# RTCartist/Neuromorphic-Spatiotemporal-Optical-Flow

Hardware: AMD Instinct MI355X
Metric: 1080p frame-pairs/sec (Farneback, HIP) (higher is better)
Workload: dtype f32

## Files before the change

neuromorphic-spatiotemporal-optical-flow_amd/csrc/farneback_iterate_x.hip:

```cpp
#include "iterate_common.h"

namespace {

typedef __attribute__((address_space(1))) unsigned long long gu64;
typedef __attribute__((address_space(1))) unsigned gu32;
typedef __attribute__((address_space(3))) int lds_int;

__device__ __forceinline__ unsigned xcc_id() { return __builtin_amdgcn_s_getreg(20 | (0 << 6) | (3 << 11)) & 7u; }

template <int MH>
struct XGeom {
    static constexpr int COLS = 208, NCW = 3, RB = 4;
    static constexpr int RL = 2 * MH + 1 + 2 * RB;
    static constexpr int HALO = 2 * MH + 1;
    static constexpr int SW = NCW * 64;
    static_assert(SW + HALO <= COLS && SW % 8 == 0, "strip geometry");
    static constexpr int NB = COLS / 64, REM = COLS % 64;
    static_assert(REM == 16, "the remainder wave maps 4 rows x 16 columns onto its 64 lanes");
    static constexpr int SEG0 = 96, SEG1 = SW - SEG0;
    static_assert(SEG0 % 8 == 0 && SEG1 % 8 == 0 && SEG0 >= SEG1 && SEG1 > 0, "segments: whole 8-column blocks, the left one not shorter");
    static constexpr int SVW = SW + 2;
    static constexpr int WAVES = NCW + 1 + 2 * NB + 1 + 1;
    static constexpr int THREADS = 64 * WAVES;
    static constexpr int CQ = 1, IOQ = 1;
    static constexpr size_t SV1_BYTES = sizeof(double) * 4 * 5 * SVW;
    static constexpr size_t SV_BYTES = 2 * SV1_BYTES;
    static constexpr size_t VI_BYTES = sizeof(double) * 2 * 4 * 5 * MH;
    static constexpr size_t JOB_BYTES = 16;
    static constexpr size_t CB_BYTES = sizeof(double) * 2 * 2 * 20;
    static constexpr size_t RING4_BYTES = sizeof(float) * 4 * RL * COLS, RING1_BYTES = sizeof(float) * RL * COLS;
    static constexpr size_t SMEM = SV_BYTES + VI_BYTES + JOB_BYTES + CB_BYTES + RING4_BYTES + RING1_BYTES;
};

struct XRing {
    float4* q;
    float* c;
    int cols;
    __device__ __forceinline__ void put(int slot, int col, const float (&M)[5]) const
    {
        q[slot * cols + col] = make_float4(M[0], M[1], M[2], M[3]);
        c[slot * cols + col] = M[4];
    }
    __device__ __forceinline__ void get(int slot, int col, float (&M)[5]) const
    {
        const float4 v = q[slot * cols + col];
        M[0] = v.x; M[1] = v.y; M[2] = v.z; M[3] = v.w;
        M[4] = c[slot * cols + col];
    }
};

constexpr unsigned X_SPIN_LIMIT = 1u << 21;

template <int MH>
__device__ __forceinline__ void x_produce(RowIn& in, float2& fl, const XRing& ring, const Planes& R0,
                                          const Planes& R1, const FlowSrc& F, int W, int H, int xc, int col, int i)
{
    constexpr int RL = XGeom<MH>::RL;
    float Mn[5];
    matrix_from(in, xc, min(i, H - 1), W, H, Mn);
    ring.put((i + MH + 1) % RL, col, Mn);
    issue_row(in, R0, R1, W, H, xc, min(i + 8, H - 1), fl);
    fl = F.fetch(min(i + 16, H - 1));
}

template <int MH>
__device__ __forceinline__ void x_rows_above(const XRing& ring, const Planes& R0, const Planes& R1, const FlowSrc& F,
                                             int W, int H, int xc, int col)
{
    float2 fl[MH];
#pragma unroll
    for (int i = 0; i < MH; i++) fl[i] = F.fetch(min(i, H - 1));
    constexpr int GRP = 4;
#pragma unroll
    for (int g0 = 0; g0 < MH; g0 += GRP) {
        RowIn t[GRP];
#pragma unroll
        for (int k = 0; k < GRP; k++)
            if (g0 + k < MH) issue_row(t[k], R0, R1, W, H, xc, min(g0 + k, H - 1), fl[g0 + k]);
#pragma unroll
        for (int k = 0; k < GRP; k++)
            if (g0 + k < MH) {
                float Mi[5];
                matrix_from(t[k], xc, min(g0 + k, H - 1), W, H, Mi);
                if (g0 + k == 0) {
#pragma unroll
                    for (int j = 0; j <= MH + 1; j++) ring.put(j, col, Mi);
                } else {
                    ring.put(g0 + k + MH + 1, col, Mi);
                }
            }
    }
}

template <int MH, int GP>
__device__ __forceinline__ void x_producer_loop(const XRing& ring, const Planes& R0, const Planes& R1,
                                                const FlowSrc& F, int W, int H, int xc, int col, int nimg)
{
    if constexpr (GP == 0) x_rows_above<MH>(ring, R0, R1, F, W, H, xc, col);
    RowIn in[2][2];
    float2 fl[2][2];
#pragma unroll
    for (int ts = 0; ts < 2; ts++)
#pragma unroll
        for (int rr = 0; rr < 2; rr++) {
            const int r = min(4 * ts + MH + 2 * GP + rr, H - 1);
            issue_row(in[ts][rr], R0, R1, W, H, xc, r, F.fetch(r));
        }
#pragma unroll
    for (int ts = 0; ts < 2; ts++)
#pragma unroll
        for (int rr = 0; rr < 2; rr++) fl[ts][rr] = F.fetch(min(4 * (ts + 2) + MH + 2 * GP + rr, H - 1));
    auto step = [&](auto tsc, int t) {
        constexpr int TS = decltype(tsc)::value;
        x_produce<MH>(in[TS][0], fl[TS][0], ring, R0, R1, F, W, H, xc, col, 4 * t + MH + 2 * GP);
        x_produce<MH>(in[TS][1], fl[TS][1], ring, R0, R1, F, W, H, xc, col, 4 * t + MH + 2 * GP + 1);
    };
    step(std::integral_constant<int, 0>{}, 0);
    __syncthreads();
    step(std::integral_constant<int, 1>{}, 1);
    __syncthreads();
    for (int t = 0; t <= nimg; t += 2) {
        step(std::integral_constant<int, 0>{}, t + 2);
        __syncthreads();
        if (t + 1 > nimg) break;
        step(std::integral_constant<int, 1>{}, t + 3);
        __syncthreads();
    }
}

template <int MH, int Q0, int NQ>
__device__ __forceinline__ void x_solve_rows(const double* sv, volatile lds_int* flag, float2* Fout, size_t fpitch, int W, int H,
                                             int x0, int nimg, double scale, int lane, int t)
{
    using G = XGeom<MH>;
    constexpr int SVW = G::SVW, NBLK = G::SW / 64;
    double g[NBLK][NQ][5];
    int us[NBLK];
#pragma unroll
    for (int b = 0; b < NBLK; b++) {
        const int col = b * 64 + lane;
        const int u = t - 1 - (col >= G::SEG0 ? 1 : 0);
        us[b] = (u >= 0 && u < nimg && x0 + col < W) ? u : -1;
        const double* p = sv + (u & 1) * (G::SV1_BYTES / sizeof(double)) + col;
#pragma unroll
        for (int q = 0; q < NQ; q++)
#pragma unroll
            for (int c = 0; c < 5; c++) g[b][q][c] = p[((q + Q0) * 5 + c) * SVW];
    }
    asm volatile("s_waitcnt lgkmcnt(0)" ::: "memory");
    if (lane == 0) *flag = t + 1;
#pragma unroll
    for (int b = 0; b < NBLK; b++) {
        if (us[b] < 0) continue;
        const int x = x0 + b * 64 + lane;
#pragma unroll
        for (int q = 0; q < NQ; q++) {
            const int yo = 4 * us[b] + q + Q0;
            const double g11 = g[b][q][0] * scale, g12 = g[b][q][1] * scale, g22 = g[b][q][2] * scale;
            const double h1 = g[b][q][3] * scale, h2 = g[b][q][4] * scale;
            const double idet = nsof_recip_normal(g11 * g22 - g12 * g12 + 1e-3);
            const float ox = (float)((g11 * h2 - g12 * h1) * idet), oy = (float)((g22 * h1 - g12 * h2) * idet);
            if (yo < H) nsof_store_stream2(reinterpret_cast<float*>(Fout + (size_t)yo * fpitch + x), ox, oy);
        }
    }
}

template <int MH>
__device__ __forceinline__ void x_remainder_loop(const XRing& ring, double* cb, const Planes& R0, const Planes& R1,
                                                 const FlowSrc& F, int W, int H, int xc, int col, int r, int nimg,
                                                 gu64* cin, gu64* cout, unsigned epoch, gu32* err, const double* sv,
                                                 volatile lds_int* ioflag, float2* Fout, size_t fpitch, int x0, double scale)
{
    const int lane = threadIdx.x & 63;
    const bool io = lane < 20;
    const int l = io ? lane : 0;
    unsigned long long g0 = 0, g1 = 0;
    auto carry_load = [&](int s) {
        const gu64* q = cin + 40 * s + 2 * l;
        asm volatile("global_load_dwordx2 %0, %2, off sc1\n\tglobal_load_dwordx2 %1, %2, off offset:8 sc1"
                     : "=&v"(g0), "=&v"(g1) : "v"(q) : "memory");
    };
    auto fetch_issue = [&](int s) {
        if (!cin || !io) return;
        carry_load(s);
    };
    bool dead = false;
    auto fetch_finish = [&](int s) {
        if (!cin || !io) return;
        asm volatile("s_waitcnt vmcnt(9)" : "+v"(g0), "+v"(g1) : : "memory");
        for (unsigned spins = 0; !dead; spins++) {
            if (__all((unsigned)(g0 >> 32) == epoch && (unsigned)(g1 >> 32) == epoch)) break;
            if (spins > X_SPIN_LIMIT ||
                ((spins & 255u) == 255u && __hip_atomic_load(err, __ATOMIC_RELAXED, __HIP_MEMORY_SCOPE_AGENT) != 0u)) {
                if (lane == 0) __hip_atomic_fetch_or(err, 1u, __ATOMIC_RELAXED, __HIP_MEMORY_SCOPE_AGENT);
                dead = true;
                break;
            }
            __builtin_amdgcn_s_sleep(8);
            carry_load(s);
            asm volatile("s_waitcnt vmcnt(0)" : "+v"(g0), "+v"(g1) : : "memory");
        }
        cb[40 + (s & 1) * 20 + l] = __hiloint2double((int)(unsigned)g1, (int)(unsigned)g0);
    };
    auto publish = [&](int s) {
        if (!cout || !io) return;
        const double S = cb[(s & 1) * 20 + l];
        const unsigned long long tag = (unsigned long long)epoch << 32;
        __hip_atomic_store(cout + 40 * s + 2 * l, tag | (unsigned)__double2loint(S), __ATOMIC_RELAXED, __HIP_MEMORY_SCOPE_AGENT);
        __hip_atomic_store(cout + 40 * s + 2 * l + 1, tag | (unsigned)__double2hiint(S), __ATOMIC_RELAXED, __HIP_MEMORY_SCOPE_AGENT);
    };
    if (r == 0) x_rows_above<MH>(ring, R0, R1, F, W, H, xc, col);
    RowIn in[2];
    float2 fl[2];
#pragma unroll
    for (int ts = 0; ts < 2; ts++) {
        const int y = min(4 * ts + MH + r, H - 1);
        issue_row(in[ts], R0, R1, W, H, xc, y, F.fetch(y));
    }
#pragma unroll
    for (int ts = 0; ts < 2; ts++) fl[ts] = F.fetch(min(4 * (ts + 2) + MH + r, H - 1));
    x_produce<MH>(in[0], fl[0], ring, R0, R1, F, W, H, xc, col, MH + r);
    __syncthreads();
    fetch_issue(0);
    x_produce<MH>(in[1], fl[1], ring, R0, R1, F, W, H, xc, col, 4 + MH + r);
    fetch_finish(0);
    __syncthreads();
    auto window = [&](auto tsc, int t) {
        constexpr int TS = decltype(tsc)::value;
        if (t >= 2) publish(t - 2);
        if (t + 1 < nimg) fetch_issue(t + 1);
        x_produce<MH>(in[TS], fl[TS], ring, R0, R1, F, W, H, xc, col, 4 * (t + 2) + MH + r);
        x_solve_rows<MH, XGeom<MH>::CQ, XGeom<MH>::IOQ>(sv, ioflag, Fout, fpitch, W, H, x0, nimg, scale, lane, t);
        if (t + 1 < nimg) fetch_finish(t + 1);
        __syncthreads();
    };
    for (int t = 0; t <= nimg; t += 2) {
        window(std::integral_constant<int, 0>{}, t);
        if (t + 1 > nimg) break;
        window(std::integral_constant<int, 1>{}, t + 1);
    }
    publish(nimg - 1);
    x_solve_rows<MH, XGeom<MH>::CQ, XGeom<MH>::IOQ>(sv, ioflag, Fout, fpitch, W, H, x0, nimg, scale, lane, nimg + 1);
}

template <int MH>
__device__ __forceinline__ void x_consumer_loop(const XRing& ring, double* sv, double* vinit, volatile lds_int* sflag, float2* Fout,
                                                size_t fpitch, int W, int H, int x0, int j, int nimg, double scale, bool strip0)
{
    using G = XGeom<MH>;
    constexpr int RL = G::RL, SVW = G::SVW, HALO = G::HALO;
    const int rb = j, ra = j + HALO;
    const int vik = j == 0 ? 0 : j - MH - 1;
    const bool vi_thread = strip0 && (j == 0 || (j >= MH + 2 && j <= 2 * MH));
    __syncthreads();
    double va[5], vb[5];
    {
        float a0[5], b0[5];
        ring.get(MH + 1, ra, a0);
        ring.get(MH + 1, rb, b0);
#pragma unroll
        for (int c = 0; c < 5; c++) {
            va[c] = (double)(a0[c] * (float)(MH + 2));
            vb[c] = (double)(b0[c] * (float)(MH + 2));
        }
#pragma unroll
        for (int i = 1; i < MH; i++) {
            ring.get(i + MH + 1, ra, a0);
            ring.get(i + MH + 1, rb, b0);
#pragma unroll
            for (int c = 0; c < 5; c++) {
                va[c] += (double)a0[c];
                vb[c] += (double)b0[c];
            }
        }
    }
    int slot_new = (2 * MH + 1) % RL;
    int slot_old = 0;
    const int x = x0 + j;
    const int lag = j >= G::SEG0 ? 1 : 0;
    double D[2][4][5];
    auto column_sums = [&](auto pc, int s) {
        constexpr int P = decltype(pc)::value;
#pragma unroll
        for (int q = 0; q < 4; q++) {
            float na[5], oa[5], nb[5], ob[5];
            ring.get(slot_new, ra, na);
            ring.get(slot_old, ra, oa);
            ring.get(slot_new, rb, nb);
            ring.get(slot_old, rb, ob);
#pragma unroll
            for (int c = 0; c < 5; c++) {
                const float da = na[c] - oa[c];
                const float db = nb[c] - ob[c];
                va[c] += (double)da;
                vb[c] += (double)db;
                D[P][q][c] = va[c] - vb[c];
            }
            if (vi_thread) {
#pragma unroll
                for (int c = 0; c < 5; c++) vinit[(((s & 1) * 4 + q) * 5 + c) * MH + vik] = vb[c];
            }
            slot_new = slot_new + 1 == RL ? 0 : slot_new + 1;
            slot_old = slot_old + 1 == RL ? 0 : slot_old + 1;
        }
    };
    auto publish = [&](auto pc, int p) {
        constexpr int P = decltype(pc)::value;
        if (p < 0 || p >= nimg) return;
        double* svj = sv + (p & 1) * (G::SV1_BYTES / sizeof(double)) + j;
#pragma unroll
        for (int q = 0; q < 4; q++)
#pragma unroll
            for (int c = 0; c < 5; c++) svj[(q * 5 + c) * SVW] = D[P][q][c];
    };
    column_sums(std::integral_constant<int, 0>{}, 0);
    if (!lag) publish(std::integral_constant<int, 0>{}, 0);
    __syncthreads();
    auto window = [&](auto pc, int t) {
        constexpr int P = decltype(pc)::value;
        const int u = t - 1 - lag;
        if (u >= 0 && u < nimg && x < W) {
            const double* svj = sv + (u & 1) * (G::SV1_BYTES / sizeof(double)) + j;
#pragma unroll
            for (int q = 0; q < G::CQ; q++) {
                const int yo = 4 * u + q;
                const double g11 = svj[(q * 5 + 0) * SVW] * scale, g12 = svj[(q * 5 + 1) * SVW] * scale;
                const double g22 = svj[(q * 5 + 2) * SVW] * scale;
                const double h1 = svj[(q * 5 + 3) * SVW] * scale, h2 = svj[(q * 5 + 4) * SVW] * scale;
                const double idet = nsof_recip_normal(g11 * g22 - g12 * g12 + 1e-3);
                const float ox = (float)((g11 * h2 - g12 * h1) * idet), oy = (float)((g22 * h1 - g12 * h2) * idet);
                if (yo < H) nsof_store_stream2(reinterpret_cast<float*>(Fout + (size_t)yo * fpitch + x), ox, oy);
            }
        }
        if (t == nimg + 1) return;
        if (t + 1 < nimg) column_sums(std::integral_constant<int, P ^ 1>{}, t + 1);
        for (int spin = 0; (sflag[0] < t + 1 || sflag[1] < t + 1) && spin < (1 << 22); spin++)
            __builtin_amdgcn_s_sleep(1);
        if (lag) publish(std::integral_constant<int, P>{}, t);
        else publish(std::integral_constant<int, P ^ 1>{}, t + 1);
        __syncthreads();
    };
    for (int t = 0; t <= nimg + 1; t += 2) {
        window(std::integral_constant<int, 0>{}, t);
        if (t + 1 > nimg + 1) break;
        window(std::integral_constant<int, 1>{}, t + 1);
    }
}

template <int MH>
__device__ __forceinline__ void x_solver_loop(const double* sv, volatile lds_int* sflag, float2* Fout, size_t fpitch, int W, int H,
                                              int x0, int nimg, double scale, int lane)
{
    using G = XGeom<MH>;
    __syncthreads();
    __syncthreads();
    for (int t = 0; t <= nimg + 1; t++) {
        x_solve_rows<MH, G::CQ + G::IOQ, 4 - G::CQ - G::IOQ>(sv, sflag, Fout, fpitch, W, H, x0, nimg, scale, lane, t);
        if (t <= nimg) __syncthreads();
    }
}

template <int MH>
__device__ __forceinline__ void x_scanner_loop(double* sv, const double* vinit, double* cb, bool has_left, int nimg, int ncols,
                                               int lane)
{
    using G = XGeom<MH>;
    constexpr int SVW = G::SVW;
    typedef double d2 __attribute__((ext_vector_type(2)));
    const int seg = lane >= 20 ? 1 : 0;
    const int l = lane < 40 ? lane - 20 * seg : 0;
    double Smid = 0.;
    __syncthreads();
    __builtin_amdgcn_s_setprio(3);
    __syncthreads();
    for (int t = 0; t <= nimg; t++) {
        const int step = t - seg;
        const double Sleft = __shfl(Smid, lane >= 20 ? lane - 20 : lane);
        d2* row = reinterpret_cast<d2*>(sv + (step & 1) * (G::SV1_BYTES / sizeof(double)) + l * SVW + seg * G::SEG0);
        if (lane < 40 && step >= 0 && step < nimg) {
            double S;
            if (seg) {
                S = Sleft;
            } else if (has_left) {
                S = cb[40 + (step & 1) * 20 + l];
            } else {
                const double* vi = vinit + ((step & 1) * 20 + l) * MH;
                S = vi[0] * (double)(MH + 2);
#pragma unroll
                for (int k = 1; k < MH; k++) S += vi[k];
            }
            auto scan_blocks = [&](int b0, int nb) {
                unsigned a = (unsigned)(size_t)(__attribute__((address_space(3))) char*)(row + 4 * b0);
                int nrem = nb - 1;
                asm volatile(
                "ds_read_b128 v[64:67], %[a]\n\t"
                "ds_read_b128 v[68:71], %[a] offset:16\n\t"
                "ds_read_b128 v[72:75], %[a] offset:32\n\t"
                "ds_read_b128 v[76:79], %[a] offset:48\n\t"
                "ds_read_b128 v[80:83], %[a] offset:64\n\t"
                "ds_read_b128 v[84:87], %[a] offset:80\n\t"
                "ds_read_b128 v[88:91], %[a] offset:96\n\t"
                "ds_read_b128 v[92:95], %[a] offset:112\n\t"
                "s_waitcnt lgkmcnt(7)\n\t"
                "v_add_f64 v[64:65], %[S], v[64:65]\n\t"
                "v_add_f64 v[66:67], v[66:67], v[64:65]\n\t"
                "s_waitcnt lgkmcnt(6)\n\t"
                "v_add_f64 v[68:69], v[66:67], v[68:69]\n\t"
                "v_add_f64 v[70:71], v[70:71], v[68:69]\n\t"
                "s_waitcnt lgkmcnt(5)\n\t"
                "v_add_f64 v[72:73], v[70:71], v[72:73]\n\t"
// ... 51 lines not shown
                "ds_write_b128 %[a], v[68:71] offset:144\n\t"
                "ds_write_b128 %[a], v[72:75] offset:160\n\t"
                "ds_write_b128 %[a], v[76:79] offset:176\n\t"
                "v_add_u32 %[a], 128, %[a]\n\t"
                "s_sub_i32 %[n], %[n], 2\n\t"
                "s_cmp_ge_i32 %[n], 2\n\t"
                "s_cbranch_scc1 .Lxs_loop%=\n"
                ".Lxs_tail%=:\n\t"
                "s_cmp_lt_i32 %[n], 1\n\t"
                "s_cbranch_scc1 .Lxs_done%=\n\t"
                "s_waitcnt lgkmcnt(4)\n\t"
                "v_add_f64 v[80:81], v[78:79], v[80:81]\n\t"
                "v_add_f64 v[82:83], v[82:83], v[80:81]\n\t"
                "s_waitcnt lgkmcnt(4)\n\t"
                "v_add_f64 v[84:85], v[82:83], v[84:85]\n\t"
                "v_add_f64 v[86:87], v[86:87], v[84:85]\n\t"
                "s_waitcnt lgkmcnt(4)\n\t"
                "v_add_f64 v[88:89], v[86:87], v[88:89]\n\t"
                "v_add_f64 v[90:91], v[90:91], v[88:89]\n\t"
                "s_waitcnt lgkmcnt(4)\n\t"
                "v_add_f64 v[92:93], v[90:91], v[92:93]\n\t"
                "v_add_f64 v[94:95], v[94:95], v[92:93]\n\t"
                "s_nop 1\n\t"
                "ds_write_b128 %[a], v[80:83] offset:64\n\t"
                "ds_write_b128 %[a], v[84:87] offset:80\n\t"
                "ds_write_b128 %[a], v[88:91] offset:96\n\t"
                "ds_write_b128 %[a], v[92:95] offset:112\n\t"
                "v_mov_b64 v[78:79], v[94:95]\n"
                ".Lxs_done%=:\n\t"
                "v_mov_b64 %[S], v[78:79]\n\t"
                "s_waitcnt lgkmcnt(0)\n\t"
                    : [S] "+v"(S), [a] "+v"(a), [n] "+s"(nrem)
                    :
                    : "memory", "scc", "v64", "v65", "v66", "v67", "v68", "v69", "v70", "v71", "v72", "v73", "v74", "v75", "v76", "v77", "v78", "v79", "v80", "v81", "v82", "v83", "v84", "v85", "v86", "v87", "v88", "v89", "v90", "v91", "v92", "v93", "v94", "v95");
            };
            const int nb0 = ncols >> 3, nba = nb0 < G::SEG1 / 8 ? nb0 : G::SEG1 / 8;
            scan_blocks(0, nba);
            if (nb0 > nba && !seg) scan_blocks(nba, nb0 - nba);
            if (seg) cb[(step & 1) * 20 + l] = S;
            else Smid = S;
        }
        __syncthreads();
    }
}

template <int MH, bool HET>
__global__ __launch_bounds__((XGeom<MH>::THREADS)) void k_iterate_x(
    const float* __restrict__ R0b, const float* __restrict__ R1b, size_t pair_stride, const float* __restrict__ flow_in,
    float* __restrict__ flow_out, int W, int H, int block_size, const nsof_het_item* __restrict__ items, int het_final,
    int n, int nstrips, unsigned long long* carry, unsigned* tickets, unsigned epoch, unsigned* err, int fault,
    const unsigned* __restrict__ xjobs)
{
    using G = XGeom<MH>;
    constexpr int SW = G::SW, COLS = G::COLS;
    extern __shared__ __attribute__((aligned(16))) unsigned char smem_x[];
    double* sv = reinterpret_cast<double*>(smem_x);
    double* vinit = reinterpret_cast<double*>(smem_x + G::SV_BYTES);
    int* job = reinterpret_cast<int*>(smem_x + G::SV_BYTES + G::VI_BYTES);
    double* cb = reinterpret_cast<double*>(smem_x + G::SV_BYTES + G::VI_BYTES + G::JOB_BYTES);
    XRing ring;
    ring.q = reinterpret_cast<float4*>(smem_x + G::SV_BYTES + G::VI_BYTES + G::JOB_BYTES + G::CB_BYTES);
    ring.c = reinterpret_cast<float*>(smem_x + G::SV_BYTES + G::VI_BYTES + G::JOB_BYTES + G::CB_BYTES + G::RING4_BYTES);
    ring.cols = COLS;
    const int tid = threadIdx.x;
    if (tid == 0) {
        const unsigned share = HET ? 0u : (unsigned)((n + 7) / 8) * (unsigned)nstrips;
        unsigned k = xcc_id();
        unsigned lim = HET ? xjobs[k] : share;
        unsigned i = __hip_atomic_fetch_add(tickets + 32 * k, 1u, __ATOMIC_RELAXED, __HIP_MEMORY_SCOPE_AGENT);
        if (__hip_atomic_load((gu32*)err, __ATOMIC_RELAXED, __HIP_MEMORY_SCOPE_AGENT) != 0u) i = 0xffffffffu, lim = 0;
        else if (i >= lim) {
            for (unsigned d = 1; d < 8 && i >= lim; d++) {
                k = (k + 1) & 7u;
                if constexpr (HET) lim = xjobs[k];
                i = __hip_atomic_fetch_add(tickets + 32 * k, 1u, __ATOMIC_RELAXED, __HIP_MEMORY_SCOPE_AGENT);
            }
        }
        if constexpr (HET) {
            const unsigned e = i < lim ? xjobs[8u + k * (unsigned)nstrips + i] : 0xffffffffu;
            job[0] = e != 0xffffffffu ? (int)(e >> 8) : -1;
            job[1] = (int)(e & 255u);
        } else {
            job[0] = i < share ? (int)((i / (unsigned)nstrips) * 8u + k) : -1;
            job[1] = (int)(i % (unsigned)nstrips);
        }
        job[2] = job[3] = 0;
    }
    __syncthreads();
    const int pair = job[0], strip = job[1];
    if (pair < 0 || pair >= n) return;
    size_t fpitch = (size_t)W;
    gu64* cbase;
    if constexpr (HET) {
        const nsof_het_item& it = items[pair];
        W = it.wk;
        H = it.hk;
        if (strip * SW >= W) return;
        R0b += it.offR;
        R1b = R0b + 5 * (size_t)W * H;
        pair_stride = 0;
        flow_in += 2 * it.offF;
        cbase = (gu64*)(carry + it.offR / 2);
        if (het_final) {
            flow_out = it.out;
            fpitch = (size_t)it.out_pitch;
        } else {
            flow_out += 2 * it.offF;
            fpitch = (size_t)W;
        }
    } else {
        if (strip * SW >= W) return;
        cbase = (gu64*)(carry + (size_t)pair * nstrips * (size_t)(((H + 3) / 4) * 40));
    }
    const int nimg = (H + 3) / 4;
    const int x0 = strip * SW;
    const size_t plane = (size_t)W * H;
    const size_t poff = HET ? 0 : (size_t)pair * pair_stride;
    const Planes R0 = planes_of(R0b + poff, plane);
    const Planes R1 = planes_of(R1b + poff, plane);
    const int wave = __builtin_amdgcn_readfirstlane(tid >> 6);
    volatile lds_int* sflag = (volatile lds_int*)(job + 2);
    if (wave < G::NCW) {
        float2* Fout = reinterpret_cast<float2*>(flow_out) + (HET ? 0 : (size_t)pair * plane);
        x_consumer_loop<MH>(ring, sv, vinit, sflag, Fout, fpitch, W, H, x0, tid, nimg, 1. / (block_size * block_size), strip == 0);
    } else if (wave == G::WAVES - 1) {
        float2* Fout = reinterpret_cast<float2*>(flow_out) + (HET ? 0 : (size_t)pair * plane);
        x_solver_loop<MH>(sv, sflag, Fout, fpitch, W, H, x0, nimg, 1. / (block_size * block_size), tid & 63);
    } else if (wave == G::NCW) {
        const int ncols = min(G::SEG0, (W - x0 + 7) & ~7);
        x_scanner_loop<MH>(sv, vinit, cb, strip > 0, nimg, ncols, tid & 63);
    } else {
        const int pw = wave - (G::NCW + 1);
        const int lane = tid & 63;
        FlowSrc F;
        F.base = reinterpret_cast<const char*>(flow_in) + (HET ? 0 : (size_t)pair * plane * 8);
        F.W = (unsigned)W;
        const bool is_io = pw == G::NB;
        const int gp = pw < G::NB ? 0 : 1;
        const int blk = pw < G::NB ? pw : pw - G::NB - 1;
        if (is_io) {
            const int col = G::NB * 64 + (lane & 15), r = lane >> 4;
            const int xc = clampi(x0 - MH - 1 + col, 0, W - 1);
            F.xc = (unsigned)xc;
            const size_t per_strip = (size_t)nimg * 40;
            gu64* cin = strip > 0 ? cbase + (size_t)(strip - 1) * per_strip : nullptr;
            gu64* cout = x0 + SW < W && !((fault & 1) && pair == 0 && strip == 0) ? cbase + (size_t)strip * per_strip : nullptr;
            float2* Fout = reinterpret_cast<float2*>(flow_out) + (HET ? 0 : (size_t)pair * plane);
            x_remainder_loop<MH>(ring, cb, R0, R1, F, W, H, xc, col, r, nimg, cin, cout, epoch, (gu32*)err, sv, sflag + 1, Fout, fpitch,
                                 x0, 1. / (block_size * block_size));
        } else {
            const int col = blk * 64 + lane;
            const int xc = clampi(x0 - MH - 1 + col, 0, W - 1);
            F.xc = (unsigned)xc;
            if (gp == 0)
                x_producer_loop<MH, 0>(ring, R0, R1, F, W, H, xc, col, nimg);
            else
                x_producer_loop<MH, 1>(ring, R0, R1, F, W, H, xc, col, nimg);
        }
    }
}

template <int MH, bool HET>
int launch_x(nsof_ctx* ctx, int n, int max_w, int max_h, const float* R0, const float* R1, size_t pair_stride,
             const float* flow_in, float* flow_out, int W, int H, int winsize, const nsof_het_item* items, bool final,
             const unsigned* xjobs, int stride, int njobs)
{
    using G = XGeom<MH>;
    static_assert(G::SW == NSOF_X_STRIP, "the host's job tables count strips of NSOF_X_STRIP columns");
    if (int rc = lds_opt_in(ctx, k_iterate_x<MH, HET>, G::SMEM)) return rc;
    const int nstrips = HET ? stride : (max_w + G::SW - 1) / G::SW;
    unsigned long long* carry = nullptr;
    unsigned* tickets = nullptr;
    unsigned* err = nullptr;
    const size_t cbytes = HET ? 0 : (size_t)n * nstrips * (size_t)((max_h + 3) / 4) * 40 * 8;
    if (int rc = nsof_xsync_reserve(ctx, cbytes, &carry, &tickets, &err)) return rc;
    NSOF_HIP(ctx, hipMemsetAsync(tickets, 0, 8 * 32 * sizeof(unsigned), ctx->stream));
    unsigned epoch = ++ctx->x_epoch;
    if (epoch == 0) {
        NSOF_HIP(ctx, hipMemsetAsync(ctx->x_carry, 0, ctx->x_carry_bytes, ctx->stream));
        epoch = ++ctx->x_epoch;
    }
    const unsigned grid = HET ? (unsigned)njobs : 8u * (unsigned)((n + 7) / 8) * (unsigned)nstrips;
    hipLaunchKernelGGL((k_iterate_x<MH, HET>), dim3(grid), dim3(G::THREADS), G::SMEM, ctx->stream, R0, R1, pair_stride, flow_in,
                       flow_out, W, H, winsize, items, final ? 1 : 0, n, nstrips, carry, tickets, epoch, err, ctx->dbg_fault,
                       xjobs);
    return NSOF_OK;
}

}

bool nsof_iterate_x_supported(int winsize, int W, int H)
{
    const int m = winsize / 2;
    return m >= 1 && m <= 7 && W >= 2 && H >= 2;
}

#define NSOF_X_SWITCH(HETV, ...)                                                                     \
    switch (winsize / 2) {                                                                           \
        case 1: rc = launch_x<1, HETV>(__VA_ARGS__); break;                                          \
        case 2: rc = launch_x<2, HETV>(__VA_ARGS__); break;                                          \
        case 3: rc = launch_x<3, HETV>(__VA_ARGS__); break;                                          \
        case 4: rc = launch_x<4, HETV>(__VA_ARGS__); break;                                          \
        case 5: rc = launch_x<5, HETV>(__VA_ARGS__); break;                                          \
        case 6: rc = launch_x<6, HETV>(__VA_ARGS__); break;                                          \
        case 7: rc = launch_x<7, HETV>(__VA_ARGS__); break;                                          \
        default: return nsof_set_error(ctx, NSOF_EUNSUPPORTED, "exact-order fused iteration supports winsize 2..15"); \
    }

int nsof_launch_iterate_x(nsof_ctx* ctx, int n_pairs, const float* R0, const float* R1, size_t pair_stride,
                          const float* flow_in, float* flow_out, int W, int H, int winsize)
{
    nsof_prof_scope ps(ctx, NSOF_K_ITERATE);
    int rc;
    NSOF_X_SWITCH(false, ctx, n_pairs, W, H, R0, R1, pair_stride, flow_in, flow_out, W, H, winsize, nullptr, false, nullptr, 0, 0)
    if (rc) return rc;
    NSOF_HIP(ctx, hipGetLastError());
    return NSOF_OK;
}

int nsof_launch_iterate_x_het(nsof_ctx* ctx, int n_items, const nsof_het_item* d_items, int max_w, int max_h, const float* R,
                              size_t R_floats, const float* flow_in, float* flow_out, bool final, int winsize,
                              const unsigned* d_xjobs, int stride, int njobs)
{
    if (njobs <= 0) return NSOF_OK;
    nsof_prof_scope ps(ctx, NSOF_K_ITERATE);
    unsigned long long* carry;
    unsigned *tk, *er;
    if (int rc0 = nsof_xsync_reserve(ctx, R_floats * 4, &carry, &tk, &er)) return rc0;
    int rc;
    NSOF_X_SWITCH(true, ctx, n_items, max_w, max_h, R, R, (size_t)0, flow_in, flow_out, 0, 0, winsize, d_items, final, d_xjobs,
                  stride, njobs)
    if (rc) return rc;
    NSOF_HIP(ctx, hipGetLastError());
    return NSOF_OK;
}
// ... 1 lines not shown
```

neuromorphic-spatiotemporal-optical-flow_amd/csrc/nsof_internal.h:

```cpp
#pragma once
#include <hip/hip_runtime.h>

#include <cstdarg>
#include <cstdio>
#include <vector>

#include "nsof.h"

#define NSOF_MAX_POLY_N 10
#define NSOF_MAX_BLUR_TAPS 64

struct nsof_prof_slot {
    std::vector<hipEvent_t> start, stop;
    size_t used = 0;
    double acc_ms = 0;
    long long acc_launches = 0;
};

struct nsof_ctx {
    int device = 0;
    hipStream_t stream = nullptr;
    hipStream_t own_stream = nullptr;
    unsigned prof_mask = 0;
    nsof_prof_slot prof[NSOF_K_COUNT];
    int opt_polyexp_f32 = 0;
    int opt_exact_rowsums = 1;
    int opt_row_bands = 0;
    int opt_small_batch_jobs = 64;
    int dbg_fault = 0;
    int opt_pyr_fma = 0;
    char err[512] = {0};
    void* ws = nullptr;
    size_t ws_bytes = 0;
    void* stage = nullptr;
    size_t stage_bytes = 0;
    void* hstage = nullptr;
    size_t hstage_bytes = 0;
    void* tmp = nullptr;
    size_t tmp_bytes = 0;
    void* het_h = nullptr;
    void* het_d = nullptr;
    size_t het_bytes = 0;
    hipEvent_t het_ev[2] = {nullptr, nullptr};
    int het_flip = 0;
    struct nsof_pipe* pipe = nullptr;
    hipStream_t side = nullptr;
    std::vector<hipEvent_t> ov_events;
    void* roi_tmp = nullptr;
    size_t roi_tmp_bytes = 0;
    void* paste_h = nullptr;
    void* paste_d = nullptr;
    size_t paste_bytes = 0;
    hipEvent_t paste_ev = nullptr;
    unsigned long long* x_carry = nullptr;
    size_t x_carry_bytes = 0;
    unsigned* x_sync = nullptr;
    unsigned x_epoch = 0;
    bool x_dirty = false;
};

int nsof_set_error(nsof_ctx* ctx, int code, const char* fmt, ...);
int nsof_ws_reserve(nsof_ctx* ctx, void** buf, size_t* cur, size_t need);
void* nsof_pinned_alloc(int device, size_t bytes);
int nsof_gpu_numa_node(int device);
int nsof_hstage_reserve(nsof_ctx* ctx, size_t need);

#define NSOF_HIP(ctx, call)                                                                      \
    do {                                                                                         \
        hipError_t e_ = (call);                                                                  \
        if (e_ != hipSuccess)                                                                    \
            return nsof_set_error((ctx), NSOF_EDEVICE, "%s failed: %s (%s:%d)", #call,           \
                                  hipGetErrorString(e_), __FILE__, __LINE__);                    \
    } while (0)

struct nsof_prof_scope {
    nsof_ctx* ctx;
    int id;
    bool on;
    nsof_prof_scope(nsof_ctx* c, int k);
    ~nsof_prof_scope();
};

enum nsof_src_type { NSOF_SRC_U8 = 0, NSOF_SRC_F32 = 1 };
int nsof_check_farneback_params(nsof_ctx* ctx, int width, int height, double pyr_scale, int levels, int winsize,
                                int iterations, int poly_n, int flags);
int nsof_farneback_core(nsof_ctx* ctx, bool sequence, int n_pairs, const void* d_prev, const void* d_next,
                        ptrdiff_t row_stride, ptrdiff_t pair_stride, int width, int height, float* d_flow,
                        double pyr_scale, int levels, int winsize, int iterations, int poly_n, double poly_sigma,
                        int flags, int src = NSOF_SRC_U8);
void nsof_pipe_destroy(nsof_ctx* ctx);

struct nsof_blur_taps {
    int ksize;
    float k[NSOF_MAX_BLUR_TAPS];
};
struct nsof_poly_taps {
    int n;
    float g[NSOF_MAX_POLY_N + 1], xg[NSOF_MAX_POLY_N + 1], xxg[NSOF_MAX_POLY_N + 1];
    double dg[NSOF_MAX_POLY_N + 1], dxxg[NSOF_MAX_POLY_N + 1];
    double ig11, ig03, ig33, ig55;
};

int nsof_host_blur_taps(int ksize, double sigma, nsof_blur_taps* out);
static inline int nsof_level_geom(nsof_ctx* ctx, int width, int height, double pyr_scale, int level, int* wk, int* hk,
                                  nsof_blur_taps* bt)
{
    int ks;
    double sg;
    int rc = nsof_farneback_level_size(width, height, pyr_scale, level, wk, hk, &ks, &sg);
    if (rc) return ctx ? nsof_set_error(ctx, rc, "bad level geometry") : rc;
// ... 96 lines not shown
```

Measured before the change: 6855.

## Make iterate-x kernel persistent with per-CU grid and pipelined job handoff

Launches one block per compute unit. Each block loops over strip jobs taken from per-XCC ticket counters, where before there was one block per job. The next job is claimed early by the solver wave into a double-buffered LDS slot. The producers prefetch the next job's above-rows and flows while the current job drains its tail, so setup cost and tail bubbles overlap with useful work. This adds control complexity and flag-epoch offsets, and the loop-tail restructuring (the tail is peeled) risks synchronisation bugs.

Result: no change. 6939 (median of 6 runs) (+1.2%).

```diff
diff --git a/neuromorphic-spatiotemporal-optical-flow_amd/csrc/farneback_iterate_x.hip b/neuromorphic-spatiotemporal-optical-flow_amd/csrc/farneback_iterate_x.hip
--- a/neuromorphic-spatiotemporal-optical-flow_amd/csrc/farneback_iterate_x.hip
+++ b/neuromorphic-spatiotemporal-optical-flow_amd/csrc/farneback_iterate_x.hip
@@ -26,7 +26,7 @@
     static constexpr size_t SV1_BYTES = sizeof(double) * 4 * 5 * SVW;
     static constexpr size_t SV_BYTES = 2 * SV1_BYTES;
     static constexpr size_t VI_BYTES = sizeof(double) * 2 * 4 * 5 * MH;
-    static constexpr size_t JOB_BYTES = 16;
+    static constexpr size_t JOB_BYTES = 32;
     static constexpr size_t CB_BYTES = sizeof(double) * 2 * 2 * 20;
     static constexpr size_t RING4_BYTES = sizeof(float) * 4 * RL * COLS, RING1_BYTES = sizeof(float) * RL * COLS;
     static constexpr size_t SMEM = SV_BYTES + VI_BYTES + JOB_BYTES + CB_BYTES + RING4_BYTES + RING1_BYTES;
@@ -51,6 +51,108 @@
 
 constexpr unsigned X_SPIN_LIMIT = 1u << 21;
 
+struct XArgs {
+    const float* R0b;
+    const float* R1b;
+    size_t pair_stride;
+    const float* flow_in;
+    float* flow_out;
+    int W, H;
+    const nsof_het_item* items;
+    int het_final, n, nstrips;
+    unsigned long long* carry;
+    unsigned* tickets;
+    unsigned* err;
+    const unsigned* xjobs;
+};
+
+struct XJob {
+    int pair, strip, W, H, nimg, x0;
+    size_t fpitch;
+    Planes R0, R1;
+    const char* fbase;
+    float2* Fout;
+    gu64* cbase;
+};
+
+template <int MH, bool HET>
+__device__ __forceinline__ bool x_job(const XArgs& A, const volatile int* slot, XJob& J)
+{
+    J.pair = __builtin_amdgcn_readfirstlane(slot[0]);
+    J.strip = __builtin_amdgcn_readfirstlane(slot[1]);
+    if (J.pair < 0) return false;
+    const float* R0b = A.R0b;
+    const float* R1b = A.R1b;
+    const float* flow_in = A.flow_in;
+    J.W = A.W;
+    J.H = A.H;
+    if constexpr (HET) {
+        const nsof_het_item& it = A.items[J.pair];
+        J.W = it.wk;
+        J.H = it.hk;
+        R0b += it.offR;
+        R1b = R0b + 5 * (size_t)J.W * J.H;
+        flow_in += 2 * it.offF;
+        J.cbase = (gu64*)(A.carry + it.offR / 2);
+        if (A.het_final) {
+            J.Fout = reinterpret_cast<float2*>(it.out);
+            J.fpitch = (size_t)it.out_pitch;
+        } else {
+            J.Fout = reinterpret_cast<float2*>(A.flow_out) + it.offF;
+            J.fpitch = (size_t)J.W;
+        }
+    } else {
+        const size_t plane = (size_t)J.W * J.H;
+        R0b += (size_t)J.pair * A.pair_stride;
+        R1b += (size_t)J.pair * A.pair_stride;
+        flow_in += 2 * (size_t)J.pair * plane;
+        J.Fout = reinterpret_cast<float2*>(A.flow_out) + (size_t)J.pair * plane;
+        J.fpitch = (size_t)J.W;
+        J.cbase = (gu64*)(A.carry + (size_t)J.pair * A.nstrips * (size_t)(((J.H + 3) / 4) * 40));
+    }
+    J.nimg = (J.H + 3) / 4;
+    J.x0 = J.strip * XGeom<MH>::SW;
+    const size_t plane = (size_t)J.W * J.H;
+    J.R0 = planes_of(R0b, plane);
+    J.R1 = planes_of(R1b, plane);
+    J.fbase = reinterpret_cast<const char*>(flow_in);
+    return true;
+}
+
+template <bool HET>
+__device__ __forceinline__ void x_take(const XArgs& A, volatile int* slot)
+{
+    auto lim_of = [&](unsigned k) -> unsigned {
+        if constexpr (HET) return A.xjobs[k];
+        return A.n > (int)k ? (unsigned)((A.n - (int)k + 7) / 8) * (unsigned)A.nstrips : 0u;
+    };
+    unsigned k = xcc_id();
+    unsigned lim = lim_of(k);
+    unsigned i = __hip_atomic_fetch_add(A.tickets + 32 * k, 1u, __ATOMIC_RELAXED, __HIP_MEMORY_SCOPE_AGENT);
+    if (__hip_atomic_load((gu32*)A.err, __ATOMIC_RELAXED, __HIP_MEMORY_SCOPE_AGENT) != 0u) {
+        i = 0xffffffffu, lim = 0;
+    } else {
+        for (unsigned d = 1; d < 8 && i >= lim; d++) {
+            k = (k + 1) & 7u;
+            lim = lim_of(k);
+            i = __hip_atomic_fetch_add(A.tickets + 32 * k, 1u, __ATOMIC_RELAXED, __HIP_MEMORY_SCOPE_AGENT);
+        }
+    }
+    int pair = -1, strip = 0;
+    if (i < lim) {
+        if constexpr (HET) {
+            const unsigned e = A.xjobs[8u + k * (unsigned)A.nstrips + i];
+            pair = (int)(e >> 8);
+            strip = (int)(e & 255u);
+        } else {
+            pair = (int)((i / (unsigned)A.nstrips) * 8u + k);
+            strip = (int)(i % (unsigned)A.nstrips);
+        }
+    }
+    slot[0] = pair;
+    slot[1] = strip;
+}
+
 template <int MH>
 __device__ __forceinline__ void x_produce(RowIn& in, float2& fl, const XRing& ring, const Planes& R0,
                                           const Planes& R1, const FlowSrc& F, int W, int H, int xc, int col, int i)
@@ -64,22 +166,28 @@
 }
 
 template <int MH>
-__device__ __forceinline__ void x_rows_above(const XRing& ring, const Planes& R0, const Planes& R1, const FlowSrc& F,
-                                             int W, int H, int xc, int col)
-{
-    float2 fl[MH];
-#pragma unroll
-    for (int i = 0; i < MH; i++) fl[i] = F.fetch(min(i, H - 1));
+__device__ __forceinline__ void x_above_flows(const FlowSrc& F, int H, float2 (&fa)[MH])
+{
+#pragma unroll
+    for (int i = 0; i < MH; i++) fa[i] = F.fetch(min(i, H - 1));
+}
+
+template <int MH, typename Mid>
+__device__ __forceinline__ void x_above_rows(const XRing& ring, const Planes& R0, const Planes& R1, int W, int H, int xc, int col,
+                                             const float2 (&fl)[MH], bool active, Mid mid)
+{
     constexpr int GRP = 4;
+    asm volatile("" : "+v"(col));
 #pragma unroll
     for (int g0 = 0; g0 < MH; g0 += GRP) {
+        if (g0 == GRP) mid();
         RowIn t[GRP];
 #pragma unroll
         for (int k = 0; k < GRP; k++)
-            if (g0 + k < MH) issue_row(t[k], R0, R1, W, H, xc, min(g0 + k, H - 1), fl[g0 + k]);
+            if (g0 + k < MH && active) issue_row(t[k], R0, R1, W, H, xc, min(g0 + k, H - 1), fl[g0 + k]);
 #pragma unroll
         for (int k = 0; k < GRP; k++)
-            if (g0 + k < MH) {
+            if (g0 + k < MH && active) {
                 float Mi[5];
                 matrix_from(t[k], xc, min(g0 + k, H - 1), W, H, Mi);
                 if (g0 + k == 0) {
@@ -90,47 +198,86 @@
                 }
             }
     }
-}
-
-template <int MH, int GP>
-__device__ __forceinline__ void x_producer_loop(const XRing& ring, const Planes& R0, const Planes& R1,
-                                                const FlowSrc& F, int W, int H, int xc, int col, int nimg)
-{
-    if constexpr (GP == 0) x_rows_above<MH>(ring, R0, R1, F, W, H, xc, col);
+    if (MH <= GRP) mid();
+}
+
+template <int MH, bool HET, int GP>
+__device__ __forceinline__ void x_producer_loop(const XRing& ring, const XArgs& A, const int* jobs, int col)
+{
+    XJob J;
+    if (!x_job<MH, HET>(A, jobs, J)) return;
+    int xc = clampi(J.x0 - MH - 1 + col, 0, J.W - 1);
+    FlowSrc F{J.fbase, (unsigned)J.W, (unsigned)xc};
     RowIn in[2][2];
     float2 fl[2][2];
-#pragma unroll
-    for (int ts = 0; ts < 2; ts++)
-#pragma unroll
-        for (int rr = 0; rr < 2; rr++) {
-            const int r = min(4 * ts + MH + 2 * GP + rr, H - 1);
-            issue_row(in[ts][rr], R0, R1, W, H, xc, r, F.fetch(r));
-        }
-#pragma unroll
-    for (int ts = 0; ts < 2; ts++)
-#pragma unroll
-        for (int rr = 0; rr < 2; rr++) fl[ts][rr] = F.fetch(min(4 * (ts + 2) + MH + 2 * GP + rr, H - 1));
-    auto step = [&](auto tsc, int t) {
-        constexpr int TS = decltype(tsc)::value;
-        x_produce<MH>(in[TS][0], fl[TS][0], ring, R0, R1, F, W, H, xc, col, 4 * t + MH + 2 * GP);
-        x_produce<MH>(in[TS][1], fl[TS][1], ring, R0, R1, F, W, H, xc, col, 4 * t + MH + 2 * GP + 1);
-    };
-    step(std::integral_constant<int, 0>{}, 0);
-    __syncthreads();
-    step(std::integral_constant<int, 1>{}, 1);
-    __syncthreads();
-    for (int t = 0; t <= nimg; t += 2) {
-        step(std::integral_constant<int, 0>{}, t + 2);
-        __syncthreads();
-        if (t + 1 > nimg) break;
-        step(std::integral_constant<int, 1>{}, t + 3);
-        __syncthreads();
+    float2 fs[2][2];
+    auto fetch01 = [&](int H) {
+#pragma unroll
+        for (int ts = 0; ts < 2; ts++)
+#pragma unroll
+            for (int rr = 0; rr < 2; rr++) fs[ts][rr] = F.fetch(min(4 * ts + MH + 2 * GP + rr, H - 1));
+    };
+    if constexpr (GP == 0) {
+        float2 fa[MH];
+        x_above_flows<MH>(F, J.H, fa);
+        x_above_rows<MH>(ring, J.R0, J.R1, J.W, J.H, xc, col, fa, true, [&] { fetch01(J.H); });
+    } else {
+        fetch01(J.H);
+    }
+    auto issue01 = [&](const XJob& K) {
+#pragma unroll
+        for (int ts = 0; ts < 2; ts++)
+#pragma unroll
+            for (int rr = 0; rr < 2; rr++) {
+                const int r = min(4 * ts + MH + 2 * GP + rr, K.H - 1);
+                issue_row(in[ts][rr], K.R0, K.R1, K.W, K.H, xc, r, fs[ts][rr]);
+            }
+#pragma unroll
+        for (int ts = 0; ts < 2; ts++)
+#pragma unroll
+            for (int rr = 0; rr < 2; rr++) fl[ts][rr] = F.fetch(min(4 * (ts + 2) + MH + 2 * GP + rr, K.H - 1));
+    };
+    issue01(J);
+    for (int jc = 0;; jc++) {
+        const int W = J.W, H = J.H, nimg = J.nimg;
+        asm volatile("" : "+v"(col));
+        auto step = [&](auto tsc, int t) {
+            constexpr int TS = decltype(tsc)::value;
+            x_produce<MH>(in[TS][0], fl[TS][0], ring, J.R0, J.R1, F, W, H, xc, col, 4 * t + MH + 2 * GP);
+            x_produce<MH>(in[TS][1], fl[TS][1], ring, J.R0, J.R1, F, W, H, xc, col, 4 * t + MH + 2 * GP + 1);
+        };
+        step(std::integral_constant<int, 0>{}, 0);
+        __syncthreads();
+        step(std::integral_constant<int, 1>{}, 1);
+        __syncthreads();
+        for (int t = 0; t <= nimg - 2; t += 2) {
+            step(std::integral_constant<int, 0>{}, t + 2);
+            __syncthreads();
+            if (t + 1 > nimg - 2) break;
+            step(std::integral_constant<int, 1>{}, t + 3);
+            __syncthreads();
+        }
+        XJob Jn;
+        const bool more = x_job<MH, HET>(A, jobs + 2 * ((jc + 1) & 1), Jn);
+        float2 fa[MH];
+        if (more) {
+            xc = clampi(Jn.x0 - MH - 1 + col, 0, Jn.W - 1);
+            F = FlowSrc{Jn.fbase, (unsigned)Jn.W, (unsigned)xc};
+            if constexpr (GP == 1) fetch01(Jn.H);
+        }
+        __syncthreads();
+        __syncthreads();
+        if (!more) return;
+        if constexpr (GP == 0) x_above_flows<MH>(F, Jn.H, fa);
+        if constexpr (GP == 0) x_above_rows<MH>(ring, Jn.R0, Jn.R1, Jn.W, Jn.H, xc, col, fa, true, [&] { fetch01(Jn.H); });
+        issue01(Jn);
+        J = Jn;
     }
 }
 
 template <int MH, int Q0, int NQ>
 __device__ __forceinline__ void x_solve_rows(const double* sv, volatile lds_int* flag, float2* Fout, size_t fpitch, int W, int H,
-                                             int x0, int nimg, double scale, int lane, int t)
+                                             int x0, int nimg, double scale, int lane, int t, int wb)
 {
     using G = XGeom<MH>;
     constexpr int SVW = G::SVW, NBLK = G::SW / 64;
@@ -148,7 +295,7 @@
             for (int c = 0; c < 5; c++) g[b][q][c] = p[((q + Q0) * 5 + c) * SVW];
     }
     asm volatile("s_waitcnt lgkmcnt(0)" ::: "memory");
-    if (lane == 0) *flag = t + 1;
+    if (lane == 0) *flag = wb + t + 1;
 #pragma unroll
     for (int b = 0; b < NBLK; b++) {
         if (us[b] < 0) continue;
@@ -165,15 +312,27 @@
     }
 }
 
-template <int MH>
-__device__ __forceinline__ void x_remainder_loop(const XRing& ring, double* cb, const Planes& R0, const Planes& R1,
-                                                 const FlowSrc& F, int W, int H, int xc, int col, int r, int nimg,
-                                                 gu64* cin, gu64* cout, unsigned epoch, gu32* err, const double* sv,
-                                                 volatile lds_int* ioflag, float2* Fout, size_t fpitch, int x0, double scale)
-{
+template <int MH, bool HET>
+__device__ __forceinline__ void x_remainder_loop(const XRing& ring, double* cb, const XArgs& A, const int* jobs, unsigned epoch,
+                                                 int fault, const double* sv, volatile lds_int* ioflag, double scale)
+{
+    using G = XGeom<MH>;
     const int lane = threadIdx.x & 63;
     const bool io = lane < 20;
     const int l = io ? lane : 0;
+    const int col = G::NB * 64 + (lane & 15);
+    int r = lane >> 4;
+    gu32* err = (gu32*)A.err;
+    XJob J;
+    if (!x_job<MH, HET>(A, jobs, J)) return;
+    int xc, nimg;
+    FlowSrc F;
+    gu64 *cin, *cout;
+    auto start = [&](const XJob& K) {
+        xc = clampi(K.x0 - MH - 1 + col, 0, K.W - 1);
+        F = FlowSrc{K.fbase, (unsigned)K.W, (unsigned)xc};
+    };
+    start(J);
     unsigned long long g0 = 0, g1 = 0;
     auto carry_load = [&](int s) {
         const gu64* q = cin + 40 * s + 2 * l;
@@ -209,43 +368,78 @@
         __hip_atomic_store(cout + 40 * s + 2 * l, tag | (unsigned)__double2loint(S), __ATOMIC_RELAXED, __HIP_MEMORY_SCOPE_AGENT);
         __hip_atomic_store(cout + 40 * s + 2 * l + 1, tag | (unsigned)__double2hiint(S), __ATOMIC_RELAXED, __HIP_MEMORY_SCOPE_AGENT);
     };
-    if (r == 0) x_rows_above<MH>(ring, R0, R1, F, W, H, xc, col);
     RowIn in[2];
     float2 fl[2];
-#pragma unroll
-    for (int ts = 0; ts < 2; ts++) {
-        const int y = min(4 * ts + MH + r, H - 1);
-        issue_row(in[ts], R0, R1, W, H, xc, y, F.fetch(y));
-    }
-#pragma unroll
-    for (int ts = 0; ts < 2; ts++) fl[ts] = F.fetch(min(4 * (ts + 2) + MH + r, H - 1));
-    x_produce<MH>(in[0], fl[0], ring, R0, R1, F, W, H, xc, col, MH + r);
-    __syncthreads();
-    fetch_issue(0);
-    x_produce<MH>(in[1], fl[1], ring, R0, R1, F, W, H, xc, col, 4 + MH + r);
-    fetch_finish(0);
-    __syncthreads();
-    auto window = [&](auto tsc, int t) {
-        constexpr int TS = decltype(tsc)::value;
-        if (t >= 2) publish(t - 2);
-        if (t + 1 < nimg) fetch_issue(t + 1);
-        x_produce<MH>(in[TS], fl[TS], ring, R0, R1, F, W, H, xc, col, 4 * (t + 2) + MH + r);
-        x_solve_rows<MH, XGeom<MH>::CQ, XGeom<MH>::IOQ>(sv, ioflag, Fout, fpitch, W, H, x0, nimg, scale, lane, t);
-        if (t + 1 < nimg) fetch_finish(t + 1);
-        __syncthreads();
-    };
-    for (int t = 0; t <= nimg; t += 2) {
-        window(std::integral_constant<int, 0>{}, t);
-        if (t + 1 > nimg) break;
-        window(std::integral_constant<int, 1>{}, t + 1);
-    }
-    publish(nimg - 1);
-    x_solve_rows<MH, XGeom<MH>::CQ, XGeom<MH>::IOQ>(sv, ioflag, Fout, fpitch, W, H, x0, nimg, scale, lane, nimg + 1);
+    float2 fs[2];
+    auto fetch01 = [&](int H) {
+#pragma unroll
+        for (int ts = 0; ts < 2; ts++) fs[ts] = F.fetch(min(4 * ts + MH + r, H - 1));
+    };
+    {
+        float2 fa[MH];
+        if (r == 0) x_above_flows<MH>(F, J.H, fa);
+        x_above_rows<MH>(ring, J.R0, J.R1, J.W, J.H, xc, col, fa, r == 0, [&] { fetch01(J.H); });
+    }
+    auto issue01 = [&](const XJob& K) {
+#pragma unroll
+        for (int ts = 0; ts < 2; ts++) issue_row(in[ts], K.R0, K.R1, K.W, K.H, xc, min(4 * ts + MH + r, K.H - 1), fs[ts]);
+#pragma unroll
+        for (int ts = 0; ts < 2; ts++) fl[ts] = F.fetch(min(4 * (ts + 2) + MH + r, K.H - 1));
+    };
+    issue01(J);
+    int wb = 0;
+    int colj = col;
+    for (int jc = 0;; jc++) {
+        const int W = J.W, H = J.H, x0 = J.x0;
+        nimg = J.nimg;
+        asm volatile("" : "+v"(colj), "+v"(r));
+        const size_t per_strip = (size_t)nimg * 40;
+        cin = J.strip > 0 ? J.cbase + (size_t)(J.strip - 1) * per_strip : nullptr;
+        cout = x0 + G::SW < W && !((fault & 1) && J.pair == 0 && J.strip == 0) ? J.cbase + (size_t)J.strip * per_strip : nullptr;
+        x_produce<MH>(in[0], fl[0], ring, J.R0, J.R1, F, W, H, xc, colj, MH + r);
+        __syncthreads();
+        fetch_issue(0);
+        x_produce<MH>(in[1], fl[1], ring, J.R0, J.R1, F, W, H, xc, colj, 4 + MH + r);
+        fetch_finish(0);
+        __syncthreads();
+        auto window = [&](auto tsc, int t) {
+            constexpr int TS = decltype(tsc)::value;
+            if (t >= 2) publish(t - 2);
+            if (t + 1 < nimg) fetch_issue(t + 1);
+            x_produce<MH>(in[TS], fl[TS], ring, J.R0, J.R1, F, W, H, xc, colj, 4 * (t + 2) + MH + r);
+            x_solve_rows<MH, G::CQ, G::IOQ>(sv, ioflag, J.Fout, J.fpitch, W, H, x0, nimg, scale, lane, t, wb);
+            if (t + 1 < nimg) fetch_finish(t + 1);
+            __syncthreads();
+        };
+        for (int t = 0; t <= nimg - 2; t += 2) {
+            window(std::integral_constant<int, 0>{}, t);
+            if (t + 1 > nimg - 2) break;
+            window(std::integral_constant<int, 1>{}, t + 1);
+        }
+        XJob Jn;
+        const bool more = x_job<MH, HET>(A, jobs + 2 * ((jc + 1) & 1), Jn);
+        float2 fa[MH];
+        if (nimg >= 3) publish(nimg - 3);
+        x_solve_rows<MH, G::CQ, G::IOQ>(sv, ioflag, J.Fout, J.fpitch, W, H, x0, nimg, scale, lane, nimg - 1, wb);
+        __syncthreads();
+        if (nimg >= 2) publish(nimg - 2);
+        x_solve_rows<MH, G::CQ, G::IOQ>(sv, ioflag, J.Fout, J.fpitch, W, H, x0, nimg, scale, lane, nimg, wb);
+        __syncthreads();
+        publish(nimg - 1);
+        x_solve_rows<MH, G::CQ, G::IOQ>(sv, ioflag, J.Fout, J.fpitch, W, H, x0, nimg, scale, lane, nimg + 1, wb);
+        if (!more) return;
+        start(Jn);
+        if (r == 0) x_above_flows<MH>(F, Jn.H, fa);
+        x_above_rows<MH>(ring, Jn.R0, Jn.R1, Jn.W, Jn.H, xc, col, fa, r == 0, [&] { fetch01(Jn.H); });
+        issue01(Jn);
+        wb += nimg + 2;
+        J = Jn;
+    }
 }
 
 template <int MH>
 __device__ __forceinline__ void x_consumer_loop(const XRing& ring, double* sv, double* vinit, volatile lds_int* sflag, float2* Fout,
-                                                size_t fpitch, int W, int H, int x0, int j, int nimg, double scale, bool strip0)
+                                                size_t fpitch, int W, int H, int x0, int j, int nimg, double scale, bool strip0, int wb)
 {
     using G = XGeom<MH>;
     constexpr int RL = G::RL, SVW = G::SVW, HALO = G::HALO;
@@ -334,7 +528,7 @@
         }
         if (t == nimg + 1) return;
         if (t + 1 < nimg) column_sums(std::integral_constant<int, P ^ 1>{}, t + 1);
-        for (int spin = 0; (sflag[0] < t + 1 || sflag[1] < t + 1) && spin < (1 << 22); spin++)
+        for (int spin = 0; (sflag[0] < wb + t + 1 || sflag[1] < wb + t + 1) && spin < (1 << 22); spin++)
             __builtin_amdgcn_s_sleep(1);
         if (lag) publish(std::integral_constant<int, P>{}, t);
         else publish(std::integral_constant<int, P ^ 1>{}, t + 1);
@@ -347,15 +541,18 @@
     }
 }
 
-template <int MH>
+template <int MH, bool HET>
 __device__ __forceinline__ void x_solver_loop(const double* sv, volatile lds_int* sflag, float2* Fout, size_t fpitch, int W, int H,
-                                              int x0, int nimg, double scale, int lane)
+                                              int x0, int nimg, double scale, int lane, int wb, const XArgs& A, volatile int* next)
 {
     using G = XGeom<MH>;
+    const int tt = max(nimg - 3, -1);
     __syncthreads();
+    if (tt == -1 && lane == 0) x_take<HET>(A, next);
     __syncthreads();
     for (int t = 0; t <= nimg + 1; t++) {
-        x_solve_rows<MH, G::CQ + G::IOQ, 4 - G::CQ - G::IOQ>(sv, sflag, Fout, fpitch, W, H, x0, nimg, scale, lane, t);
+        x_solve_rows<MH, G::CQ + G::IOQ, 4 - G::CQ - G::IOQ>(sv, sflag, Fout, fpitch, W, H, x0, nimg, scale, lane, t, wb);
+        if (t == tt && lane == 0) x_take<HET>(A, next);
         if (t <= nimg) __syncthreads();
     }
 }
@@ -513,111 +710,52 @@
     const unsigned* __restrict__ xjobs)
 {
     using G = XGeom<MH>;
-    constexpr int SW = G::SW, COLS = G::COLS;
     extern __shared__ __attribute__((aligned(16))) unsigned char smem_x[];
     double* sv = reinterpret_cast<double*>(smem_x);
     double* vinit = reinterpret_cast<double*>(smem_x + G::SV_BYTES);
-    int* job = reinterpret_cast<int*>(smem_x + G::SV_BYTES + G::VI_BYTES);
+    int* jobs = reinterpret_cast<int*>(smem_x + G::SV_BYTES + G::VI_BYTES);
     double* cb = reinterpret_cast<double*>(smem_x + G::SV_BYTES + G::VI_BYTES + G::JOB_BYTES);
     XRing ring;
     ring.q = reinterpret_cast<float4*>(smem_x + G::SV_BYTES + G::VI_BYTES + G::JOB_BYTES + G::CB_BYTES);
     ring.c = reinterpret_cast<float*>(smem_x + G::SV_BYTES + G::VI_BYTES + G::JOB_BYTES + G::CB_BYTES + G::RING4_BYTES);
-    ring.cols = COLS;
+    ring.cols = G::COLS;
+    const XArgs A{R0b, R1b, pair_stride, flow_in, flow_out, W, H, items, het_final, n, nstrips, carry, tickets, err, xjobs};
     const int tid = threadIdx.x;
     if (tid == 0) {
-        const unsigned share = HET ? 0u : (unsigned)((n + 7) / 8) * (unsigned)nstrips;
-        unsigned k = xcc_id();
-        unsigned lim = HET ? xjobs[k] : share;
-        unsigned i = __hip_atomic_fetch_add(tickets + 32 * k, 1u, __ATOMIC_RELAXED, __HIP_MEMORY_SCOPE_AGENT);
-        if (__hip_atomic_load((gu32*)err, __ATOMIC_RELAXED, __HIP_MEMORY_SCOPE_AGENT) != 0u) i = 0xffffffffu, lim = 0;
-        else if (i >= lim) {
-            for (unsigned d = 1; d < 8 && i >= lim; d++) {
-                k = (k + 1) & 7u;
-                if constexpr (HET) lim = xjobs[k];
-                i = __hip_atomic_fetch_add(tickets + 32 * k, 1u, __ATOMIC_RELAXED, __HIP_MEMORY_SCOPE_AGENT);
+        x_take<HET>(A, jobs);
+        jobs[4] = jobs[5] = 0;
+    }
+    __syncthreads();
+    const int wave = __builtin_amdgcn_readfirstlane(tid >> 6);
+    volatile lds_int* sflag = (volatile lds_int*)(jobs + 4);
+    const double scale = 1. / (block_size * block_size);
+    if (wave < G::NCW || wave == G::WAVES - 1 || wave == G::NCW) {
+        int wb = 0;
+        for (int jc = 0;; jc++) {
+            XJob J;
+            if (!x_job<MH, HET>(A, jobs + 2 * (jc & 1), J)) return;
+            int th = tid;
+            asm volatile("" : "+v"(th));
+            if (wave < G::NCW) {
+                x_consumer_loop<MH>(ring, sv, vinit, sflag, J.Fout, J.fpitch, J.W, J.H, J.x0, th, J.nimg, scale, J.strip == 0, wb);
+            } else if (wave == G::WAVES - 1) {
+                x_solver_loop<MH, HET>(sv, sflag, J.Fout, J.fpitch, J.W, J.H, J.x0, J.nimg, scale, th & 63, wb, A,
+                                       jobs + 2 * ((jc + 1) & 1));
+            } else {
+                const int ncols = min(G::SEG0, (J.W - J.x0 + 7) & ~7);
+                x_scanner_loop<MH>(sv, vinit, cb, J.strip > 0, J.nimg, ncols, th & 63);
             }
-        }
-        if constexpr (HET) {
-            const unsigned e = i < lim ? xjobs[8u + k * (unsigned)nstrips + i] : 0xffffffffu;
-            job[0] = e != 0xffffffffu ? (int)(e >> 8) : -1;
-            job[1] = (int)(e & 255u);
-        } else {
-            job[0] = i < share ? (int)((i / (unsigned)nstrips) * 8u + k) : -1;
-            job[1] = (int)(i % (unsigned)nstrips);
-        }
-        job[2] = job[3] = 0;
-    }
-    __syncthreads();
-    const int pair = job[0], strip = job[1];
-    if (pair < 0 || pair >= n) return;
-    size_t fpitch = (size_t)W;
-    gu64* cbase;
-    if constexpr (HET) {
-        const nsof_het_item& it = items[pair];
-        W = it.wk;
-        H = it.hk;
-        if (strip * SW >= W) return;
-        R0b += it.offR;
-        R1b = R0b + 5 * (size_t)W * H;
-        pair_stride = 0;
-        flow_in += 2 * it.offF;
-        cbase = (gu64*)(carry + it.offR / 2);
-        if (het_final) {
-            flow_out = it.out;
-            fpitch = (size_t)it.out_pitch;
-        } else {
-            flow_out += 2 * it.offF;
-            fpitch = (size_t)W;
-        }
+            wb += J.nimg + 2;
+        }
+    }
+    const int pw = wave - (G::NCW + 1);
+    const int lane = tid & 63;
+    if (pw == G::NB) {
+        x_remainder_loop<MH, HET>(ring, cb, A, jobs, epoch, fault, sv, sflag + 1, scale);
+    } else if (pw < G::NB) {
+        x_producer_loop<MH, HET, 0>(ring, A, jobs, pw * 64 + lane);
     } else {
-        if (strip * SW >= W) return;
-        cbase = (gu64*)(carry + (size_t)pair * nstrips * (size_t)(((H + 3) / 4) * 40));
-    }
-    const int nimg = (H + 3) / 4;
-    const int x0 = strip * SW;
-    const size_t plane = (size_t)W * H;
-    const size_t poff = HET ? 0 : (size_t)pair * pair_stride;
-    const Planes R0 = planes_of(R0b + poff, plane);
-    const Planes R1 = planes_of(R1b + poff, plane);
-    const int wave = __builtin_amdgcn_readfirstlane(tid >> 6);
-    volatile lds_int* sflag = (volatile lds_int*)(job + 2);
-    if (wave < G::NCW) {
-        float2* Fout = reinterpret_cast<float2*>(flow_out) + (HET ? 0 : (size_t)pair * plane);
-        x_consumer_loop<MH>(ring, sv, vinit, sflag, Fout, fpitch, W, H, x0, tid, nimg, 1. / (block_size * block_size), strip == 0);
-    } else if (wave == G::WAVES - 1) {
-        float2* Fout = reinterpret_cast<float2*>(flow_out) + (HET ? 0 : (size_t)pair * plane);
-        x_solver_loop<MH>(sv, sflag, Fout, fpitch, W, H, x0, nimg, 1. / (block_size * block_size), tid & 63);
-    } else if (wave == G::NCW) {
-        const int ncols = min(G::SEG0, (W - x0 + 7) & ~7);
-        x_scanner_loop<MH>(sv, vinit, cb, strip > 0, nimg, ncols, tid & 63);
-    } else {
-        const int pw = wave - (G::NCW + 1);
-        const int lane = tid & 63;
-        FlowSrc F;
-        F.base = reinterpret_cast<const char*>(flow_in) + (HET ? 0 : (size_t)pair * plane * 8);
-        F.W = (unsigned)W;
-        const bool is_io = pw == G::NB;
-        const int gp = pw < G::NB ? 0 : 1;
-        const int blk = pw < G::NB ? pw : pw - G::NB - 1;
-        if (is_io) {
-            const int col = G::NB * 64 + (lane & 15), r = lane >> 4;
-            const int xc = clampi(x0 - MH - 1 + col, 0, W - 1);
-            F.xc = (unsigned)xc;
-            const size_t per_strip = (size_t)nimg * 40;
-            gu64* cin = strip > 0 ? cbase + (size_t)(strip - 1) * per_strip : nullptr;
-            gu64* cout = x0 + SW < W && !((fault & 1) && pair == 0 && strip == 0) ? cbase + (size_t)strip * per_strip : nullptr;
-            float2* Fout = reinterpret_cast<float2*>(flow_out) + (HET ? 0 : (size_t)pair * plane);
-            x_remainder_loop<MH>(ring, cb, R0, R1, F, W, H, xc, col, r, nimg, cin, cout, epoch, (gu32*)err, sv, sflag + 1, Fout, fpitch,
-                                 x0, 1. / (block_size * block_size));
-        } else {
-            const int col = blk * 64 + lane;
-            const int xc = clampi(x0 - MH - 1 + col, 0, W - 1);
-            F.xc = (unsigned)xc;
-            if (gp == 0)
-                x_producer_loop<MH, 0>(ring, R0, R1, F, W, H, xc, col, nimg);
-            else
-                x_producer_loop<MH, 1>(ring, R0, R1, F, W, H, xc, col, nimg);
-        }
+        x_producer_loop<MH, HET, 1>(ring, A, jobs, (pw - G::NB - 1) * 64 + lane);
     }
 }
 
@@ -641,7 +779,9 @@
         NSOF_HIP(ctx, hipMemsetAsync(ctx->x_carry, 0, ctx->x_carry_bytes, ctx->stream));
         epoch = ++ctx->x_epoch;
     }
-    const unsigned grid = HET ? (unsigned)njobs : 8u * (unsigned)((n + 7) / 8) * (unsigned)nstrips;
+    if (ctx->x_cus <= 0) NSOF_HIP(ctx, hipDeviceGetAttribute(&ctx->x_cus, hipDeviceAttributeMultiprocessorCount, ctx->device));
+    const long long jobs = HET ? (long long)njobs : (long long)n * nstrips;
+    const unsigned grid = (unsigned)std::min<long long>(jobs, std::max(ctx->x_cus, 1));
     hipLaunchKernelGGL((k_iterate_x<MH, HET>), dim3(grid), dim3(G::THREADS), G::SMEM, ctx->stream, R0, R1, pair_stride, flow_in,
                        flow_out, W, H, winsize, items, final ? 1 : 0, n, nstrips, carry, tickets, epoch, err, ctx->dbg_fault,
                        xjobs);
diff --git a/neuromorphic-spatiotemporal-optical-flow_amd/csrc/nsof_internal.h b/neuromorphic-spatiotemporal-optical-flow_amd/csrc/nsof_internal.h
--- a/neuromorphic-spatiotemporal-optical-flow_amd/csrc/nsof_internal.h
+++ b/neuromorphic-spatiotemporal-optical-flow_amd/csrc/nsof_internal.h
@@ -56,6 +56,7 @@
     size_t x_carry_bytes = 0;
     unsigned* x_sync = nullptr;
     unsigned x_epoch = 0;
+    int x_cus = 0;
     bool x_dirty = false;
 };
 
```
